# richarddurbin/modimizer

Hardware: AMD Instinct MI355X
Metric: Gbp/s hashed+sketched (k=21,d=64) (higher is better)
Workload: dtype u64; 1 GPU; BASELINE config 2: 10 Gbp synthetic ONT-like reads (log-normal N50 20 kb, 5% subs, 30x of a 333 Mbp genome), k=21 d=64 seed=17, seqhash scan + modset build (table bits 30); reads_per_gpu=598835, bases_per_gpu=10000000000, modimizers_per_gpu=156043826, modset_entries=102967436, k=21, d=64, table_bits=30, parallelism=reads sharded x1, modset per GPU

## Files before the change

### modimizer_amd/csrc/mg_api.hip

```cpp
#include <stdarg.h>
#include <stdlib.h>
#include <string.h>
#include <mutex>
#include <unordered_map>
#include "mg_common.h"
#include "mg_internal.h"
#include "mg_xfer.h"


static thread_local char gErr[512] = "";

void mgSetError (const char *fmt, ...)
{ va_list ap; va_start (ap, fmt); vsnprintf (gErr, sizeof (gErr), fmt, ap); va_end (ap); }

extern "C" const char *mgLastError (void) { return gErr; }

MgStatus mgHipFail (hipError_t e, const char *what)
{ mgSetError ("HIP error %d (%s) in %s", (int) e, hipGetErrorString (e), what); return MG_ERR_HIP; }

extern "C" int mgDeviceCount (void)
{ int n = 0; if (hipGetDeviceCount (&n) != hipSuccess) { (void) hipGetLastError (); return 0; } return n; }

MgStatus mgEnsureDevice (void)
{
// ... 430 lines not shown
static std::unordered_map<const Modset *, MgDev *> gReg;
extern "C" { volatile int mgLiveDeviceModsets = 0; }

static MgDev *mgDevLookup (const Modset *ms)
{ std::lock_guard<std::mutex> g (gRegLock); auto it = gReg.find (ms); return it == gReg.end () ? 0 : it->second; }

static void mgDevFree (MgDev *d)
{
  if (!d) return;
  MgOnDevice here (d->device);
  if (d->hPin) (void) hipHostFree (d->hPin);
  if (d->built)
    { (void) hipFree (d->t.slots); (void) hipFree (d->t.value); (void) hipFree (d->t.occ); (void) hipFree (d->t.find8);
      (void) hipFree (d->t.baseDepth); (void) hipFree (d->t.counters); (void) hipFree (d->t.liveHist);
    }
  if (d->side) { (void) hipStreamSynchronize (d->side); (void) hipStreamDestroy (d->side); }
  d->arena.release (); d->arena2.release ();
  for (int i = 0 ; i < 2 ; ++i) if (d->scanned[i]) (void) hipEventDestroy (d->scanned[i]);
  if (d->inputReady) (void) hipEventDestroy (d->inputReady);
  delete d;
}

#define MG_LOOKUP_LOAD_PCT 40
static MgStatus mgDevBuild (Modset *ms, MgDev *d, hipStream_t st)
{
  MgTable &t = d->t;
  if (ms->tableBits < 20 || ms->tableBits > 32)
    { mgSetError ("device modset supports table bits 20..32 (got %d)", ms->tableBits); return MG_ERR_ARG; }
  memset (&t, 0, sizeof (t));
  t.maxLog2Slots = ms->tableBits - 1;
  t.kbits = 2 * ms->hasher->k;
  t.wantR = 4096;
  { const long r = mgKnobs ()->bucketR; if (r != MG_KNOB_UNSET && r >= 256) t.wantR = (U32) r; }
  t.size = ms->size;
  t.pin = d->hPin + 24;
  U64 cap = (ms->tableSize >> 2);
  MG_HIP (hipMalloc ((void **) &t.value, cap * sizeof (U64)));
  MG_HIP (hipMalloc ((void **) &t.baseDepth, cap * sizeof (U16)));
  MG_HIP (hipMalloc ((void **) &t.counters, 64));
  d->built = true;
  MG_HIP (hipMemsetAsync (t.baseDepth, 0, cap * sizeof (U16), st));
  MG_HIP (hipMemsetAsync (t.counters, 0, 64, st));
  { MgStatus s0 = mgTableEnsure (&t, ms->max, st); if (s0) return s0; }
  t.max = 0; t.syncedMax = 0;
  t.baseZero = !ms->max;
  if (ms->max)
    { MG_HIP (hipStreamSynchronize (st));
      MgStatus s;
      if ((s = mgXferH2D (t.value, ms->value, ((size_t) ms->max + 1) * sizeof (U64)))) return s;
      if ((s = mgXferH2D (t.baseDepth, ms->depth, ((size_t) ms->max + 1) * sizeof (U16)))) return s;
      if ((s = mgTableLoadHost (&t, t.value, 1, ms->max, st))) return s;
      MG_HIP (hipStreamSynchronize (st));
      t.max = t.syncedMax = ms->max;
    }
  d->hostIndexMax = ms->max;
// ... 208 lines not shown

static U64 mgAddChunkSize (void)
{
  const long c = mgKnobs ()->addChunk;
  U64 v = c != MG_KNOB_UNSET && c > 0 ? (U64) c : ((U64) 1 << 30);
  if (v > ((U64) 1 << 30)) v = (U64) 1 << 30;
  return v;
}
#define MG_ADD_CHUNK (mgAddChunkSize ())

static MgStatus mgAddChunk (Modset *ms, MgDev *d, const U64 *dKmer, U64 n, U32 *dIndexOut, int withDepth,
                            void *scratch, hipStream_t st, const MgHistReq *counted = 0, const MgSegSrc *segSrc = 0)
{
  MgTable &t = d->t;
  MgStatus s;
  MG_HIP (hipMemsetAsync (t.counters, 0, 16, st));
  if ((s = mgTableAdd (&t, dKmer, n, withDepth, scratch, st, counted, segSrc))) return s;
  volatile U64 *c = d->hPin;
  MG_HIP (hipMemcpyAsync (d->hPin, t.counters, 16, hipMemcpyDeviceToHost, st));
  MG_HIP (hipStreamSynchronize (st));
  U64 newMax = (U64) t.max + c[0];
  if (c[1] || newMax >= t.size)
    {
      if ((s = mgTableRollback (&t, st))) return s;
      mgSetError ("hashTableSize %u is too small for %llu", t.size, (unsigned long long) newMax);
      return MG_ERR_CAPACITY;
    }
  t.max = (U32) newMax;
  ms->max = t.max;
  if (n >= 4096) t.newPct = (int) (c[0] * 100 / n);
  if (dIndexOut && (s = mgTableFind (&t, dKmer, n, dIndexOut, st))) return s;
// ... 634 lines not shown
```

### modimizer_amd/csrc/mg_common.h

```cpp
#ifndef MG_COMMON_H
#define MG_COMMON_H
#include "mg_knobs.h"

#include <hip/hip_runtime.h>
#include <stdint.h>
#include <time.h>
#include <algorithm>
#include <vector>
#include "modgpu.h"

#define MG_WAVE 64

#define MG_SCAN_THREADS   256
#define MG_POS_PER_THREAD 64
#define MG_TILE_BASES     (64 * MG_POS_PER_THREAD)
#define MG_TILE_WORDS     (MG_TILE_BASES / 16)

struct MgHashParams {
  U64 factor1;
  U64 mask;
  int k;
  int shift1;
  U32 d;
  int dShift;
// ... 184 lines not shown
  U32 syncedMax;
  U64 *counters;
  bool pendingDepth;
  bool dirty;
  U64 *find8;
  U64 find8Cap;
  U64 find8Version, version;
  bool empty;
  U64 *pin;
  int newPct;
  int loadPct;
  int  maxLog2Slots;
  U32  wantR;
  U64  diag[7];
  int  tightPct;
};
MgStatus mgTableAlloc (MgTable *t, U64 slotsWanted, hipStream_t st);
MgStatus mgTableEnsure (MgTable *t, U64 nIncoming, hipStream_t st);
MgStatus mgTableRollback (MgTable *t, hipStream_t st);
MgStatus mgTableClean (MgTable *t, hipStream_t st);
void     mgTableForget (MgTable *t, hipStream_t st);
size_t   mgTableAddScratchBytes (const MgTable *t, U64 n);
bool     mgTableUseBuckets (const MgTable *t, U64 n);
MgStatus mgTableAdd (MgTable *t, const U64 *dKmer, U64 n, int withDepth, void *scratch, hipStream_t st,
                     const MgHistReq *counted = 0,
                     const MgSegSrc *segSrc = 0);
bool     mgTableAddTakesSegments (const MgTable *t, U64 n, const MgHistReq *counted);
MgStatus mgTableMarkOccupied (MgTable *t, const U64 *dKmer, U64 n, hipStream_t st);
MgStatus mgTableFind (MgTable *t, const U64 *dKmer, U64 n, U32 *dIndexOut, hipStream_t st);
MgStatus mgTableLayoutCheck (MgTable *t, U64 *dOut4, hipStream_t st);
enum { MG_DIAG_FIND_DIRECT = 0, MG_DIAG_FIND_PART1, MG_DIAG_FIND_PART2_16, MG_DIAG_FIND_PART2_8, MG_DIAG_PACK8, MG_DIAG_REHASH_BUCKET, MG_DIAG_REHASH_ATOMIC };
// ... 24 lines not shown
```

### modimizer_amd/csrc/mg_knobs.c

```c
#define _GNU_SOURCE
#include <pthread.h>
#include <sched.h>
#include <stdio.h>
#include <stdlib.h>
#include <string.h>
#include <unistd.h>
#include <sys/mman.h>
#include "mg_knobs.h"

static MgKnobs gKnobs;
static pthread_once_t gOnce = PTHREAD_ONCE_INIT;

static long num (const char *name)
{ const char *e = getenv (name); return e && *e ? atol (e) : MG_KNOB_UNSET; }

static void readAll (void)
{
  MgKnobs k;
  const char *e = getenv ("MODGPU_TABLE_PATH");
  k.tablePath = e && *e ? (long) e[0] : MG_KNOB_UNSET;
  e = getenv ("MODGPU_FIND_PATH");
  k.findPath = e && *e ? (long) e[0] : MG_KNOB_UNSET;
  k.partPacked = num ("MODGPU_PART_PACKED");       k.partBig = num ("MODGPU_PART_BIG");
  k.addChunk = num ("MODGPU_ADD_CHUNK");           k.scanGrid = num ("MODGPU_SCAN_GRID");
  k.scanGeneric = num ("MODGPU_SCAN_GENERIC");     k.scanHist = num ("MODGPU_SCAN_HIST");
  k.scanDiv64 = num ("MODGPU_SCAN_DIV64");        k.minTiled = num ("MODGPU_MIN_TILED");
  k.minTile = num ("MODGPU_MIN_TILE");
  k.noSegmentInput = num ("MODGPU_NO_SEGMENT_INPUT");
  k.rankSliceShift = num ("MODGPU_RANK_SLICE_SHIFT");
  k.flagPolarity = num ("MODGPU_FLAG_POLARITY");   k.mergeSlots = num ("MODGPU_MERGE_SLOTS");
  k.mergePlace = num ("MODGPU_MERGE_PLACE");
  k.bucketR = num ("MODGPU_BUCKET_R");             k.bucketT = num ("MODGPU_BUCKET_T");
  e = getenv ("MODGPU_HOT_SPLIT");
  k.hotSplit = e && *e ? atol (e) : MG_KNOB_UNSET;
  { const char *c = e ? strchr (e, ',') : 0; k.hotChunk = c ? atol (c + 1) : MG_KNOB_UNSET; }
  k.noAvx2 = num ("MODGPU_NO_AVX2");               k.textHost = num ("MODGPU_TEXT_HOST");
  k.textWindowKb = num ("MODGPU_TEXT_WINDOW_KB");
  k.fileBatchMbp = num ("MODGPU_FILE_BATCH_MBP");  k.fileBatchBases = num ("MODGPU_FILE_BATCH_BASES");
  k.queryHostChain = num ("MODGPU_QUERY_HOST_CHAIN");
  k.iterHostBelow = num ("MODGPU_ITER_HOST_BELOW");
  k.readsetHost = num ("MODGPU_READSET_HOST");
  k.segSlack = num ("MODGPU_SEG_SLACK");
  k.partDigits = num ("MODGPU_PART_DIGITS");
  k.findBits = num ("MODGPU_FIND_BITS");
  k.scatterGrid = num ("MODGPU_SCATTER_GRID");     k.tableLoad = num ("MODGPU_TABLE_LOAD");
  k.tightLoad = num ("MODGPU_TIGHT_LOAD");         k.find8 = num ("MODGPU_FIND8");
// ... 44 lines not shown
```

### modimizer_amd/csrc/mg_knobs.h

```cpp
#ifndef MG_KNOBS_H
#define MG_KNOBS_H
#include <limits.h>
#ifdef __cplusplus
extern "C" {
#endif
#define MG_KNOB_UNSET LONG_MIN
typedef struct {
  long findPath;
  long tablePath;
  long partPacked;
  long partBig;
  long addChunk;
  long scanGrid;
  long scanGeneric;
  long minTile;
  long minTiled;
  long scanDiv64;
  long scanHist;
  long noSegmentInput;
  long rankSliceShift;
  long flagPolarity;
  long mergeSlots;
  long mergePlace;
  long bucketR, bucketT;
  long hotSplit, hotChunk;
  long noAvx2;
  long textHost;
  long textWindowKb;
  long fileBatchMbp;
  long fileBatchBases;
  long readsetHost;
  long queryHostChain;
  long iterHostBelow;
  long scatterGrid;
  long segSlack;
  long partDigits;
  long findBits;
  long tableLoad;
// ... 22 lines not shown
```

### modimizer_amd/csrc/mg_scan.hip

```cpp
#include <stdlib.h>
#include "mg_prefix.h"


__global__ void mgPackKernel (const U8 *__restrict__ bases, U64 nBases, U32 *__restrict__ words, U64 nWords)
{
  U64 i = (U64) blockIdx.x * blockDim.x + threadIdx.x;
  U64 stride = (U64) gridDim.x * blockDim.x;
  const bool aligned = (((uintptr_t) bases) & 15) == 0;
  for ( ; i < nWords ; i += stride)
    { U64 b0 = i * 16;
      U32 w = 0;
      if (b0 + 16 <= nBases && aligned)
        { uint4 v = *reinterpret_cast<const uint4 *> (bases + b0);
          U32 q[4] = { v.x, v.y, v.z, v.w };
#pragma unroll
          for (int j = 0 ; j < 4 ; ++j)
            { U32 x = q[j];
              U32 n = ((x & 3) << 6) | (((x >> 8) & 3) << 4) | (((x >> 16) & 3) << 2) | ((x >> 24) & 3);
              w |= n << (24 - 8 * j);
            }
        }
      else if (b0 < nBases)
        { for (int j = 0 ; j < 16 && b0 + j < nBases ; ++j)
            w |= (U32) (bases[b0 + j] & 3) << (30 - 2 * j);
// ... 466 lines not shown
  for (int w = 0 ; w < MG_ITER_WAVES ; ++w) { const U64 v = sFound[w]; if (w < wave) before += v; total += v; }
  if (total <= o.capEntries)
    { U32 *posOut = reinterpret_cast<U32 *> (o.out + 1 + total);
      const U64 src = (U64) wave * a.segCap;
      for (U64 i = (U64) lane ; i < found ; i += 64)
        { o.out[1 + before + i] = a.segKmer[src + i];
          posOut[before + i] = a.segPosF[src + i];
        }
    }
  if (threadIdx.x == 0) o.out[0] = total;
  __threadfence_system ();
  __syncthreads ();
  if (threadIdx.x == 0) __hip_atomic_store (const_cast<U64 *> (o.flag), o.seq, __ATOMIC_RELEASE, __HIP_MEMORY_SCOPE_SYSTEM);
}

__global__ __launch_bounds__ (1024)
void mgSegScanKernel (const U64 *__restrict__ blockCount, U32 nBlocks, U64 segCap, U64 capacity,
                      U64 *__restrict__ segStart, U64 *__restrict__ dCount)
{
  __shared__ U64 sV[8192 + 1024];
  __shared__ U64 sWaveSum[16], sWaveMax[16];
  const int tid = threadIdx.x, lane = tid & 63, wave = tid >> 6;
  U64 carry = 0, gmx = 0;
  for (U32 base = 0 ; base < nBlocks ; base += 8192)
    {
#pragma unroll
      for (int j = 0 ; j < 8 ; ++j)
        { U32 e = (U32) j * 1024 + tid, b = base + e;
          sV[e + (e >> 3)] = b < nBlocks ? blockCount[b] : 0;
        }
      __syncthreads ();
      U64 c[8], sum = 0, mx = 0;
#pragma unroll
      for (int j = 0 ; j < 8 ; ++j) { c[j] = sV[tid * 9 + j]; sum += c[j]; if (c[j] > mx) mx = c[j]; }
      U64 incl = sum, wmx = mx;
#pragma unroll
      for (int off = 1 ; off < 64 ; off <<= 1)
        { U32 lo = __shfl_up ((U32) incl, off), hi = __shfl_up ((U32) (incl >> 32), off);
          if (lane >= off) incl += ((U64) hi << 32) | lo;
          U32 ml = __shfl_xor ((U32) wmx, off), mh = __shfl_xor ((U32) (wmx >> 32), off);
          U64 o = ((U64) mh << 32) | ml; if (o > wmx) wmx = o;
        }
      if (lane == 63) { sWaveSum[wave] = incl; sWaveMax[wave] = wmx; }
      __syncthreads ();
      U64 before = 0, total = 0;
#pragma unroll
      for (int w = 0 ; w < 16 ; ++w) { U64 v = sWaveSum[w]; if (w < wave) before += v; total += v; if (sWaveMax[w] > gmx) gmx = sWaveMax[w]; }
      U64 run = carry + before + incl - sum;
#pragma unroll
      for (int j = 0 ; j < 8 ; ++j) { sV[tid * 9 + j] = run; run += c[j]; }
      __syncthreads ();
#pragma unroll
      for (int j = 0 ; j < 8 ; ++j)
        { U32 e = (U32) j * 1024 + tid, b = base + e;
          if (b < nBlocks) segStart[b] = sV[e + (e >> 3)];
        }
      carry += total;
      __syncthreads ();
    }
  if (tid == 0)
    { segStart[nBlocks] = carry;
      dCount[0] = carry;
      dCount[1] = (gmx > segCap || carry > capacity) ? 1 : 0;
      dCount[2] = gmx;
      U64 need = gmx * (U64) nBlocks;
      dCount[3] = need > carry ? need : carry;
    }
}

__global__ __launch_bounds__ (256)
void mgSegCompactKernel (const U64 *__restrict__ segKmer, const U32 *__restrict__ segPosF,
                         const U32 *__restrict__ segRead, U64 segCap, U32 nSegs,
                         const U64 *__restrict__ blockCount, const U64 *__restrict__ segStart,
// ... 152 lines not shown
  const bool scanCounts = histEnv && hist && hist->binCount && hist->kbits >= 24 && hHiB >= 1 && hHiB <= MG_MIX_TOP && hLoB + hHiB == hist->log2NB;
  a.histCount = scanCounts ? hist->binCount : 0; a.histKbits = hist ? hist->kbits : 64; a.histHiB = hHiB;
#ifdef MG_ABLATE
  { const long dbg = mgKnobs ()->scanDebug; a.debug = dbg != MG_KNOB_UNSET ? (U32) dbg : 0u; }
#endif
  const unsigned grid = (g.nBlocks + MG_WAVES - 1) / MG_WAVES;
  const int mode = mgScanMode (p, &a);
  const bool where = a.segPosF || a.segRead;
#define MG_SCAN_LAUNCH(M) do { if (where) MG_LAUNCH (MG_K_SCAN, st, (mgScanKernel<M, true>), dim3 (grid), dim3 (MG_SCAN_THREADS), 0, st, a); \
                               else       MG_LAUNCH (MG_K_SCAN, st, (mgScanKernel<M, false>), dim3 (grid), dim3 (MG_SCAN_THREADS), 0, st, a); } while (0)
  if (mode == MG_MODE_FAST) MG_SCAN_LAUNCH (MG_MODE_FAST); else if (mode == MG_MODE_POW2) MG_SCAN_LAUNCH (MG_MODE_POW2);
  else if (mode == MG_MODE_ODD) MG_SCAN_LAUNCH (MG_MODE_ODD); else if (mode == MG_MODE_ODD32) MG_SCAN_LAUNCH (MG_MODE_ODD32);
  else if (mode == MG_MODE_ANY32) MG_SCAN_LAUNCH (MG_MODE_ANY32); else MG_SCAN_LAUNCH (MG_MODE_ANY);
#undef MG_SCAN_LAUNCH
  MG_HIP (hipGetLastError ());
  MG_LAUNCH (MG_K_SEG_SCAN, st, mgSegScanKernel, dim3 (1), dim3 (1024), 0, st, blockCount, g.nBlocks, g.segCap, capacity, segStart, dCount);
  MG_HIP (hipGetLastError ());
  { int hiB = 0, loB = 0; U32 bins = 0;
    if (hist && hist->binCount && !scanCounts) { mgPartSplit (hist->log2NB, &hiB, &loB); bins = (U32) 1 << hiB; }
    const unsigned cgrid = g.nBlocks < 4096 ? g.nBlocks : 4096;
    if (lazy) { lazy->segKmer = segKmer; lazy->segCount = blockCount; lazy->segStart = segStart; lazy->segCap = g.segCap; lazy->nSegs = g.nBlocks; }
    if (!lazy || bins || dPosF || dReadId)
      MG_LAUNCH (MG_K_SEG_COMPACT, st, mgSegCompactKernel, dim3 (cgrid), dim3 (256), 0, st,
                 segKmer, a.segPosF, a.segRead, g.segCap, g.nBlocks, blockCount, segStart, lazy ? (U64 *) 0 : dKmer, dPosF, dReadId, capacity, dCount,
                 hist ? hist->log2NB : 0, hist ? hist->kbits : 64, loB, bins, hist ? hist->binCount : (U32 *) 0);
  }
  MG_HIP (hipGetLastError ());
  return MG_OK;
}

MgStatus mgLaunchSegCompact (const MgSegSrc &src, U64 *dKmer, U64 capacity, const U64 *dCount, hipStream_t st)
// ... 55 lines not shown
```

### modimizer_amd/csrc/mg_table.hip

```cpp
#include <stdlib.h>
#include <string.h>
#include "mg_prefix.h"

#define MG_ASSIGNED 0x80000000u
#define MG_R_QUANTUM 64u
#ifdef MG_BUILD_PRIO
#define MG_BUILD_PRIO() __builtin_amdgcn_s_setprio (3)
#else
#define MG_BUILD_PRIO() do { } while (0)
#endif
#ifdef MG_ABLATE
#define MG_ABLATE_AND(x) && (x)
#else
#define MG_ABLATE_AND(x)
#endif
__device__ __forceinline__ U32 mgToken (U64 o) { return 0x7fffffffu - (U32) o; }
__device__ __forceinline__ bool mgIsAssigned (U32 v) { return (v & MG_ASSIGNED) != 0; }
__device__ __forceinline__ U64 mgKeyOf (const uint4 &v) { return ((U64) v.y << 32) | v.x; }
__device__ __forceinline__ U32 mgIndexOf (U32 ordWord) { return mgIsAssigned (ordWord) ? (ordWord & ~MG_ASSIGNED) : 0; }
__device__ __forceinline__ bool mgLiveEntry (const uint4 &v, U32 keepMax) { return (v.x | v.y) && mgIsAssigned (v.z) && (v.z & ~MG_ASSIGNED) <= keepMax; }




// ... 702 lines not shown
          if (dOut) dOut[at] = (unsigned char) mgDigitOf<(PACKOUT ? MG_EL_PACKED : MG_EL_WIDE)> (stK[p], g, f, dShift, dMask);
        }
      __syncthreads ();
      c = nc; seg = nseg; lo = nlo; hi = nhi; sub = nsub; have = nhave;
    }
}



struct MgBucketArgs {
  MgSlot *slots; MgGeom g; U32 nBuckets;
  const U64 *bucketStart;
  U64 *pK; U32 *pT; U32 *pC;
  MgPartFmt f;
  U32 *uniqCount;
  U32 *occ;
  unsigned char *flags;
  const MgRankGrp *grp; U32 baseMax; U32 size;
  unsigned short *sliceOff;
  U32 nSlices; int sliceShift;
  int slotShift;
  int place;
  int markDup;
  int withDepth;
  U64 *counters;
  U32 hotSplit, hotChunk;
  U64 *hotItems; unsigned long long *hotCount;
  U32 *hotBuckets;
#ifdef MG_ABLATE
  int debug;
// ... 240 lines not shown
    }
}

template <bool PACKED, bool SLOT, int PER, bool HOT>
__global__ __launch_bounds__ (1024) __attribute__ ((amdgpu_waves_per_eu (PER == MG_DEDUP_PER ? 8 : 4)))
void mgBucketDedupKernel (const MgBucketArgs a, U32 bucketsPerBlock)
{
  MG_BUILD_PRIO ();
  const U32 R = a.g.R, T = blockDim.x, tid = threadIdx.x;
  unsigned long long *sKey = reinterpret_cast<unsigned long long *> (mgDynLds);
  U32 *sOrd = reinterpret_cast<U32 *> (mgDynLds + (size_t) R * 8);
  U32 *sCnt = sOrd + R;
  U32 *sGrp = sCnt + R;
  const U32 nGrp = a.nSlices + 1;
  U32 b = blockIdx.x * bucketsPerBlock, bEnd = b + bucketsPerBlock;
  U64 hotAt = blockIdx.x; const U64 nHot = HOT ? a.hotCount[1] : 0;
  if (HOT) { if (hotAt >= nHot) return; }
  else
    { if (bEnd > a.nBuckets) bEnd = a.nBuckets;
      if (b >= bEnd) return;
    }
  for (U32 i = tid ; i < R ; i += T) { sKey[i] = 0; sOrd[i] = 0; sCnt[i] = 0; }
  if (tid < MG_RANK_GROUPS) sGrp[tid] = 0;
  for ( ; ; )
  {
  if (HOT) { b = a.hotBuckets[hotAt]; bEnd = b + 1; }
  U64 lo = a.bucketStart[b], hi = a.bucketStart[b + 1];
  U32 occNow = a.occ[b];
  U64 ck[MG_BUCKET_PREFETCH]; U32 ct[MG_BUCKET_PREFETCH];
#pragma unroll
// ... 55 lines not shown
              rk[j] = 0; rc[j] = 0; ro[j] = 0; rp[j] = 0;
              if (i < R) rk[j] = sKey[i];
              if (rk[j])
                { rc[j] = sCnt[i]; ro[j] = sOrd[i];
                  sKey[i] = 0; sOrd[i] = 0; sCnt[i] = 0;
                  rk[j] = (rk[j] - 1) | (SLOT ? (unsigned long long) i << MG_SLOT_SHIFT : 0ull);
                  if (rc[j]) rp[j] = atomicAdd (&sGrp[mgIsAssigned (ro[j]) ? a.nSlices : ((0x7fffffffu - ro[j]) >> a.sliceShift)], 1u);
                }
            }
          __syncthreads ();
          const int lane = (int) (tid & 63);
          const U32 gv = (U32) lane < nGrp ? sGrp[lane] : 0;
          const U32 gIncl = mgWaveInclusiveSum (gv);
          const U32 gBase = gIncl - gv;
          const U32 total = (U32) __builtin_amdgcn_readlane ((int) gIncl, 63);
          if (tid < 64)
            { if ((U32) lane <= nGrp) a.sliceOff[(U64) b * (nGrp + 1) + lane] = (unsigned short) gBase;
              if (lane == 0) a.uniqCount[b] = total;
            }
#pragma unroll
          for (int j = 0 ; j < PER ; ++j)
            { const U32 grp = mgIsAssigned (ro[j]) ? a.nSlices : ((0x7fffffffu - ro[j]) >> a.sliceShift);
              const U32 at = (U32) __shfl ((int) gBase, (int) (rc[j] ? grp : 0)) + rp[j];
              if (rc[j]) { sKey[at] = rk[j]; sOrd[at] = ro[j]; sCnt[at] = rc[j]; }
            }
          __syncthreads ();
          if (tid < MG_RANK_GROUPS) sGrp[tid] = 0;
          for (U32 i = tid ; i < total ; i += T)
            { const U64 k = sKey[i]; const U32 ord = sOrd[i], c = sCnt[i];
              sKey[i] = 0; sOrd[i] = 0; sCnt[i] = 0;
              if (true MG_ABLATE_AND (!(a.debug & 8)))
                { __builtin_nontemporal_store (k, &a.pK[lo + i]); __builtin_nontemporal_store (ord, &a.pT[lo + i]); __builtin_nontemporal_store (c, &a.pC[lo + i]); }
              if (!a.markDup && !mgIsAssigned (ord) MG_ABLATE_AND (!(a.debug & 1))) a.flags[0x7fffffffu - ord] = 1;
            }
          __syncthreads ();
        }
      lo = nlo; hi = nhi; occNow = occNext;
#pragma unroll
      for (int j = 0 ; j < MG_BUCKET_PREFETCH ; ++j) { ck[j] = nk[j]; ct[j] = nt[j]; }
    }
  if (!HOT) break;
  hotAt += gridDim.x;
  if (hotAt >= nHot) break;
  }
}

__device__ __forceinline__ U32 mgPlaceStarts (U32 *cnt, unsigned short *sStart, int *sWave, U32 R, U32 T, U32 tid, U32 n)
{
  const U32 per = (R + 4 * T - 1) / (4 * T) * 4;
  const U32 j0 = tid * per, j1 = j0 + per < R ? j0 + per : R;
  U32 vS = 0; int vM = 0;
  for (U32 j = j0 ; j < j1 ; j += 4)
    { const uint4 c = *reinterpret_cast<const uint4 *> (&cnt[j]);
      int m = (int) j - (int) vS;               vM = m > vM ? m : vM; vS += c.x;
      m = (int) (j + 1) - (int) vS;             vM = m > vM ? m : vM; vS += c.y;
      m = (int) (j + 2) - (int) vS;             vM = m > vM ? m : vM; vS += c.z;
      m = (int) (j + 3) - (int) vS;             vM = m > vM ? m : vM; vS += c.w;
    }
  const int lane = (int) (tid & 63);
// ... 826 lines not shown
#undef MG_SCATTER_P
#undef MG_SCATTER
  MG_HIP (hipGetLastError ());
  return MG_OK;
}

__global__ __launch_bounds__ (256)
void mgUniqStatsKernel (const U32 *__restrict__ uniqCount, U32 nBuckets, unsigned long long *__restrict__ out)
{
  unsigned long long sum = 0; U32 mx = 0;
  for (U32 b = blockIdx.x * 256 + threadIdx.x ; b < nBuckets ; b += gridDim.x * 256) { const U32 c = uniqCount[b]; sum += c; mx = c > mx ? c : mx; }
  sum = mgWaveReduce<MgSum> ((U64) sum); mx = mgWaveReduce<MgMax> (mx);
  if ((threadIdx.x & 63) == 0) { if (sum) atomicAdd (&out[0], sum); if (mx) atomicMax (&out[1], (unsigned long long) mx); }
}

#define MG_TIGHT_PCT_DEFAULT 70
#define MG_TIGHT_PCT_CLAIMS 50
#define MG_TIGHT_MIN_R 1024u

MgStatus mgTableAdd (MgTable *t, const U64 *dKmer, U64 n, int withDepth, void *scratch, hipStream_t st,
                     const MgHistReq *counted, const MgSegSrc *segSrc)
{
  if (!n) return MG_OK;
  if (segSrc && !mgTableAddTakesSegments (t, n, counted)) { mgSetError ("internal: this insert needs the dense k-mers"); return MG_ERR_ARG; }
  const MgSegSrc noSrc = {};
  t->liveHistValid = false;
  if (withDepth) t->pendingDepth = true;
  const bool wasEmpty = t->empty && t->max == 0;
  t->empty = false; ++t->version;
  MgGeom g = mgGeomOf (t);
  char *wb = (char *) scratch;
  unsigned char *flags = (unsigned char *) wb;       wb += mgAl256 (n);
  U64 *blockCount = (U64 *) wb;                      wb += mgAl256 ((MG_RANK_UNITS + 8) * 8);
  U64 *blockBase = (U64 *) wb;                       wb += mgAl256 ((MG_RANK_UNITS + 8) * 8);
  MgRankGrp *grp = (MgRankGrp *) wb;                 wb += mgAl256 ((n / 64 + 2) * sizeof (MgRankGrp));
  U32 nRankBlocks; U64 rankTiles = mgRankRowsPerUnit (n, &nRankBlocks);
  MG_HIP (hipMemsetAsync (blockCount, 0, (MG_RANK_UNITS + 8) * 8, st));

  if (!mgTableUseBuckets (t, n))
    { U32 *slotId = (U32 *) wb;
      { MgStatus cs = mgTableClean (t, st); if (cs) return cs; }
      MG_LAUNCH (MG_K_TABLE_INSERT, st, mgTableInsertKernel, dim3 (mgGridWide (n)), dim3 (256), 0, st, t->slots, g, dKmer, n, slotId, withDepth, t->counters);
      MG_LAUNCH (MG_K_TABLE_FLAG, st, mgDirectFlagKernel, dim3 (mgGridWide (n)), dim3 (256), 0, st, t->slots, slotId, n, flags);
      MG_LAUNCH (MG_K_RANK_COUNT, st, mgRankCountKernel, dim3 (nRankBlocks), dim3 (256), 0, st, flags, n, rankTiles, blockCount);
      MG_LAUNCH (MG_K_RANK_SCAN, st, (mgGroupSumKernel<U64, U64>), dim3 (1), dim3 (MG_GROUP_THREADS), 0, st, blockCount, blockBase, nRankBlocks * 4, t->counters);
      MG_LAUNCH (MG_K_TABLE_ASSIGN, st, (mgRankAssignKernel<true, false>), dim3 (nRankBlocks), dim3 (256), 0, st,
                 flags, dKmer, noSrc, (const MgSubSeg *) 0, n, rankTiles, blockBase, t->max, t->size, t->value, t->slots, slotId, grp);
      MG_HIP (hipGetLastError ());
      return mgTableMarkOccupied (t, dKmer, n, st);
    }

  const U64 NB = (U64) 1 << t->log2NB;
// ... 11 lines not shown
  unsigned long long *coarseCursor = (unsigned long long *) wb; wb += mgAl256 (((U64) MG_PART_MAXBINS + 2) * 8 * 16);
  U64 *whole = (U64 *) wb;                    wb += mgAl256 (((U64) MG_PART_MAXBINS + 2) * 8);
  U32 *coarseCount = (U32 *) wb;              wb += mgAl256 ((MG_PART_MAXBINS + 2) * 4);
  U32 *chunkBase = (U32 *) wb;                wb += mgAl256 ((MG_PART_MAXBINS + 2 + n / MG_PART_CHUNK + MG_PART_MAXBINS + 2) * 4);
  unsigned short *sliceOff = (unsigned short *) wb;   wb += mgAl256 ((size_t) (MG_RANK_GROUPS + 2) * NB * sizeof (unsigned short));
  MgSubSeg *subSeg = (MgSubSeg *) wb;         wb += mgAl256 ((n / MG_PART_SUB + 2) * sizeof (MgSubSeg));
  U64 *hotItems = (U64 *) wb;                 wb += mgAl256 (mgHotItemsCap (n) * 8);
  U32 *hotBuckets = (U32 *) wb;               wb += mgAl256 (mgHotItemsCap (n) * 4);
  unsigned long long *hotCount = (unsigned long long *) wb; wb += 256;
  (void) spare64;

  const int j = t->log2NB;
  int hiB, loB;
  mgPartSplit (j, &hiB, &loB);
  const U32 *pre = (counted && counted->binCount && counted->log2NB == j && counted->kbits == t->kbits && !counted->hiB) ? counted->binCount : 0;
  U64 segInit[2] = { 0, n };
  MG_HIP (hipMemcpyAsync (whole, segInit, 16, hipMemcpyHostToDevice, st));
  const MgPartFmt f = mgPartFmtOf (t, n, hiB);
  const int packEnv = mgKnobs ()->partPacked == MG_KNOB_UNSET ? 1 : (int) mgKnobs ()->partPacked;
  const bool packed = packEnv && mgPartFmtFits (t, f);
  MgStatus s;
  const U64 *bucketStart = fineStart;
  MgPartPassArgs p1 = {};
  p1.inMode = segSrc ? MG_EL_SEG : MG_EL_DENSE; p1.packed = packed; p1.f = f; p1.kIn = dKmer; p1.n = n; p1.segStart = whole; p1.nSeg = 1;
  p1.nBins = (U32) 1 << hiB; p1.chunkBase = chunkBase; p1.counted = pre; p1.segSrc = segSrc; p1.subSeg = subSeg;
  if (!loB)
    { p1.kOut = kB; p1.tOut = tB; p1.binStart = fineStart; p1.cursor = fineCursor; p1.binCount = fineCount;
      if ((s = mgPartPass (t, p1, st))) return s;
    }
  else
    {
      unsigned char *digits = (loB <= 8 && mgKnobs ()->partDigits != 0) ? reinterpret_cast<unsigned char *> (cB) : 0;
      p1.shift = loB; p1.kOut = kA; p1.tOut = tA; p1.binStart = coarseStart; p1.cursor = coarseCursor; p1.binCount = coarseCount;
      p1.digitOut = digits; p1.nextBins = (U32) 1 << loB;
      if ((s = mgPartPass (t, p1, st))) return s;
      MgPartPassArgs p2 = {};
      p2.inMode = packed ? MG_EL_PACKED : MG_EL_WIDE; p2.packed = packed; p2.f = f; p2.kIn = kA; p2.tIn = tA; p2.n = n; p2.segStart = coarseStart; p2.nSeg = (U32) 1 << hiB;
      p2.nBins = (U32) 1 << loB; p2.kOut = kB; p2.tOut = tB; p2.binStart = fineStart; p2.cursor = fineCursor; p2.binCount = fineCount; p2.chunkBase = chunkBase;
      p2.digitIn = digits;
      if ((s = mgPartPass (t, p2, st))) return s;
    }

  MgBucketArgs a;
  { const int polEnv = mgKnobs ()->flagPolarity == MG_KNOB_UNSET ? -1 : (int) mgKnobs ()->flagPolarity;
    a.markDup = polEnv >= 0 ? (polEnv ? 1 : 0) : (t->newPct > 50 ? 1 : 0);
  }
  MG_HIP (hipMemsetAsync (flags, a.markDup ? 1 : 0, n, st));
  const U64 expectNew = t->newPct > 0 ? n * (U64) t->newPct / 100 : n;
  { const int slotEnv = mgKnobs ()->mergeSlots == MG_KNOB_UNSET ? -1 : (int) mgKnobs ()->mergeSlots;
    const bool dense = ((U64) t->max + expectNew) * 2 > t->nSlots;
    a.slotShift = (t->kbits <= MG_SLOT_SHIFT && (slotEnv >= 0 ? slotEnv != 0 : dense)) ? MG_SLOT_SHIFT : 0;
  }
  int tightPct = t->tightPct ? t->tightPct : MG_TIGHT_PCT_CLAIMS;
  { const long tk = mgKnobs ()->tightLoad; if (tk != MG_KNOB_UNSET && tk >= 0 && tk <= 95) tightPct = (int) tk; }
  bool tighten = wasEmpty && tightPct > 0 && t->log2NB > 0 && t->pin;
  if (tighten && mgKnobs ()->tightLoad == MG_KNOB_UNSET)
    tighten = expectNew * 100 / (U64) tightPct < t->nSlots - t->nSlots / 4;
  { const long pk = mgKnobs ()->mergePlace;
// ... 8 lines not shown
  if (tighten) a.slotShift = 0;
  a.slots = t->slots; a.g = g; a.nBuckets = (U32) NB; a.bucketStart = bucketStart;
  a.pK = kB; a.pT = tB; a.pC = cB; a.uniqCount = uniqCount; a.occ = t->occ; a.flags = flags;
  a.grp = grp; a.baseMax = t->max; a.size = t->size; a.withDepth = withDepth;
  { a.sliceShift = 22;
    while (a.sliceShift > 16 && ((n - 1) >> a.sliceShift) + 1 < 32) --a.sliceShift;
    if (mgKnobs ()->rankSliceShift != MG_KNOB_UNSET) a.sliceShift = (int) mgKnobs ()->rankSliceShift;
    while (((n - 1) >> a.sliceShift) + 1 > (U64) (MG_RANK_GROUPS - 1)) ++a.sliceShift;
    a.nSlices = (U32) (((n - 1) >> a.sliceShift) + 1);
    a.sliceOff = sliceOff;
  }
  a.counters = t->counters; a.f = f;
#ifdef MG_ABLATE
  { const long dbg = mgKnobs ()->bucketDebug; a.debug = dbg != MG_KNOB_UNSET ? (int) dbg : 0; }
#endif
  const bool track = t->max == 0 && t->baseZero;
  a.liveHist = 0;
  if (track)
    { if (!t->liveHist) MG_HIP (hipMalloc ((void **) &t->liveHist, 65536 * sizeof (U64)));
      MG_HIP (hipMemsetAsync (t->liveHist, 0, 65536 * sizeof (U64), st));
      a.liveHist = (unsigned long long *) t->liveHist;
    }
  t->liveHistValid = track;
  size_t lds = mgMergeLdsBytes (t->R);
  { const size_t ldsDedup = (size_t) t->R * 16 + MG_RANK_GROUPS * 4; if (ldsDedup > lds) lds = ldsDedup; }
  const bool bigR = t->R > MG_DEDUP_PER * 1024u;
  if (t->R > MG_DEDUP_PER_BIG * 1024u) { mgSetError ("internal: bucket of %u slots", t->R); return MG_ERR_ARG; }
  if (lds > 48 * 1024)
    {
#define MG_DEDUP_ATTR(PK, SL, PER) do { MG_HIP (hipFuncSetAttribute ((const void *) mgBucketDedupKernel<PK, SL, PER, false>, hipFuncAttributeMaxDynamicSharedMemorySize, (int) lds)); \
                                        MG_HIP (hipFuncSetAttribute ((const void *) mgBucketDedupKernel<PK, SL, PER, true>, hipFuncAttributeMaxDynamicSharedMemorySize, (int) lds)); } while (0)
      if (bigR) { MG_DEDUP_ATTR (true, true, MG_DEDUP_PER_BIG); MG_DEDUP_ATTR (true, false, MG_DEDUP_PER_BIG); MG_DEDUP_ATTR (false, true, MG_DEDUP_PER_BIG); MG_DEDUP_ATTR (false, false, MG_DEDUP_PER_BIG); }
      else      { MG_DEDUP_ATTR (true, true, MG_DEDUP_PER); MG_DEDUP_ATTR (true, false, MG_DEDUP_PER); MG_DEDUP_ATTR (false, true, MG_DEDUP_PER); MG_DEDUP_ATTR (false, false, MG_DEDUP_PER); }
#undef MG_DEDUP_ATTR
      MG_HIP (hipFuncSetAttribute ((const void *) mgBucketMergeKernel<MG_MERGE_PREFETCH>, hipFuncAttributeMaxDynamicSharedMemorySize, (int) lds));
      MG_HIP (hipFuncSetAttribute ((const void *) mgBucketMergeKernel<MG_PLACE_KEEP>, hipFuncAttributeMaxDynamicSharedMemorySize, (int) lds));
    }
  const int bThreadsEnv = mgKnobs ()->bucketT == MG_KNOB_UNSET ? 0 : (int) mgKnobs ()->bucketT;
  const unsigned bThreads = mgBucketThreads (t->R, bThreadsEnv);
  U32 perBlock;
  const unsigned bGrid = mgBucketGrid (NB, &perBlock);
  if ((U64) bThreads * (bigR ? MG_DEDUP_PER_BIG : MG_DEDUP_PER) < t->R)
    { mgSetError ("internal: %u threads for a bucket of %u slots", bThreads, t->R); return MG_ERR_ARG; }
  mgHotKnobs (&a.hotSplit, &a.hotChunk);
  a.hotItems = hotItems; a.hotCount = hotCount; a.hotBuckets = hotBuckets;
  MG_HIP (hipMemsetAsync (hotCount, 0, 16, st));
  MG_LAUNCH (MG_K_HOT_REDUCE, st, mgHotPlanKernel, dim3 ((unsigned) ((NB + 255) / 256)), dim3 (256), 0, st, a);
  { const size_t ldsHot = (size_t) t->R * 16 + 16;
    if (packed) { if (ldsHot > 48 * 1024) MG_HIP (hipFuncSetAttribute ((const void *) mgHotReduceKernel<true>, hipFuncAttributeMaxDynamicSharedMemorySize, (int) ldsHot));
                  MG_LAUNCH (MG_K_HOT_REDUCE, st, mgHotReduceKernel<true>, dim3 (1024), dim3 (bThreads), ldsHot, st, a); }
    else        { if (ldsHot > 48 * 1024) MG_HIP (hipFuncSetAttribute ((const void *) mgHotReduceKernel<false>, hipFuncAttributeMaxDynamicSharedMemorySize, (int) ldsHot));
                  MG_LAUNCH (MG_K_HOT_REDUCE, st, mgHotReduceKernel<false>, dim3 (1024), dim3 (bThreads), ldsHot, st, a); }
  }
#define MG_DEDUP_LAUNCH(PK, SL, PER) do { MG_LAUNCH (MG_K_BUCKET_DEDUP, st, (mgBucketDedupKernel<PK, SL, PER, false>), dim3 (bGrid), dim3 (bThreads), lds, st, a, perBlock); \
                                          MG_LAUNCH (MG_K_HOT_REDUCE, st, (mgBucketDedupKernel<PK, SL, PER, true>), dim3 (64), dim3 (bThreads), lds, st, a, perBlock); } while (0)
#define MG_DEDUP_PICK(PER) do { if (packed) { if (a.slotShift) MG_DEDUP_LAUNCH (true, true, PER); else MG_DEDUP_LAUNCH (true, false, PER); } \
                                else        { if (a.slotShift) MG_DEDUP_LAUNCH (false, true, PER); else MG_DEDUP_LAUNCH (false, false, PER); } } while (0)
  if (bigR) MG_DEDUP_PICK (MG_DEDUP_PER_BIG); else MG_DEDUP_PICK (MG_DEDUP_PER);
#undef MG_DEDUP_PICK
#undef MG_DEDUP_LAUNCH
  U64 fullest = t->R;
  if (tighten)
    { unsigned long long *st2 = (unsigned long long *) (t->counters + 2);
      MG_HIP (hipMemsetAsync (st2, 0, 16, st));
      MG_LAUNCH (MG_K_RANK_SCAN, st, mgUniqStatsKernel, dim3 ((unsigned) (NB / 256 < 256 ? (NB + 255) / 256 : 256)), dim3 (256), 0, st, uniqCount, (U32) NB, st2);
      MG_HIP (hipMemcpyAsync (t->pin, t->counters + 1, 24, hipMemcpyDeviceToHost, st));
      MG_HIP (hipStreamSynchronize (st));
      const U64 over = t->pin[0], U = t->pin[1], M = t->pin[2];
      if (!over)
        { fullest = M;
          U64 Rn = (U * 100 / ((U64) NB * (U64) tightPct) + 1 + MG_R_QUANTUM - 1) / MG_R_QUANTUM * MG_R_QUANTUM;
          const U64 Rfit = (M + M / 8 + 16 + MG_R_QUANTUM - 1) / MG_R_QUANTUM * MG_R_QUANTUM;
          if (Rn < Rfit) Rn = Rfit;
          if (Rn < MG_TIGHT_MIN_R) Rn = MG_TIGHT_MIN_R;
          if (Rn < t->R)
            { t->R = (U32) Rn; t->nSlots = (U64) NB * Rn; a.g = mgGeomOf (t);
              lds = mgMergeLdsBytes (t->R);
            }
        }
    }
  MG_LAUNCH (MG_K_RANK_COUNT, st, mgRankCountKernel, dim3 (nRankBlocks), dim3 (256), 0, st, flags, n, rankTiles, blockCount);
  MG_LAUNCH (MG_K_RANK_SCAN, st, (mgGroupSumKernel<U64, U64>), dim3 (1), dim3 (MG_GROUP_THREADS), 0, st, blockCount, blockBase, nRankBlocks * 4, t->counters);
  if (segSrc)
    MG_LAUNCH (MG_K_TABLE_ASSIGN, st, (mgRankAssignKernel<false, true>), dim3 (nRankBlocks), dim3 (256), 0, st,
               flags, (const U64 *) 0, *segSrc, subSeg, n, rankTiles, blockBase, t->max, t->size, t->value, t->slots, (const U32 *) 0, grp);
  else
    MG_LAUNCH (MG_K_TABLE_ASSIGN, st, (mgRankAssignKernel<false, false>), dim3 (nRankBlocks), dim3 (256), 0, st,
               flags, dKmer, noSrc, (const MgSubSeg *) 0, n, rankTiles, blockBase, t->max, t->size, t->value, t->slots, (const U32 *) 0, grp);
  { const U32 groupsPerSlice = (U32) ((NB + 63) / 64);
    const U32 blocksPerSlice = (groupsPerSlice + 3) / 4, rounds = (a.nSlices + 7) / 8;
    MG_LAUNCH (MG_K_RANK_LOOKUP, st, mgRankLookupKernel, dim3 (8 * rounds * blocksPerSlice), dim3 (256), 0, st, a, groupsPerSlice);
  }
  if (fullest <= (U64) MG_MERGE_PREFETCH * bThreads)
    MG_LAUNCH (MG_K_BUCKET_MERGE, st, mgBucketMergeKernel<MG_MERGE_PREFETCH>, dim3 (bGrid), dim3 (bThreads), lds, st, a, perBlock);
  else
    MG_LAUNCH (MG_K_BUCKET_MERGE, st, mgBucketMergeKernel<MG_PLACE_KEEP>, dim3 (bGrid), dim3 (bThreads), lds, st, a, perBlock);
  MG_HIP (hipGetLastError ());
  return MG_OK;
}

__global__ void mgMarkOccKernel (MgGeom g, const U64 *__restrict__ kmer, U64 n, U32 *__restrict__ occ)
{
  U64 o = (U64) blockIdx.x * blockDim.x + threadIdx.x;
// ... 357 lines not shown
```

Measured before the change: 1239 Gbp/s.

## Chain modset build launches: fuse init memsets, overlap host sync with rank pass

Adds a buildChain knob that, when set, replaces several small memsets and an H2D copy with one init kernel. It folds unique-count stats into the dedup kernel instead of a separate stats kernel. It also launches the rank pass before waiting on an event for the pinned stats, so the host sync overlaps GPU work. The segment scan kernel gains a prefetching, grouped variant. The knob defaults to unset, which is nonzero, so the chained path runs by default. The cost is more code paths, and the rank pass now runs before R is tightened; this is valid only if it does not depend on R.

```diff
diff --git a/modimizer_amd/csrc/mg_api.hip b/modimizer_amd/csrc/mg_api.hip
--- a/modimizer_amd/csrc/mg_api.hip
+++ b/modimizer_amd/csrc/mg_api.hip
@@ -468,6 +468,7 @@
     { (void) hipFree (d->t.slots); (void) hipFree (d->t.value); (void) hipFree (d->t.occ); (void) hipFree (d->t.find8);
       (void) hipFree (d->t.baseDepth); (void) hipFree (d->t.counters); (void) hipFree (d->t.liveHist);
     }
+  mgTableSyncDrop (&d->t);
   if (d->side) { (void) hipStreamSynchronize (d->side); (void) hipStreamDestroy (d->side); }
   d->arena.release (); d->arena2.release ();
   for (int i = 0 ; i < 2 ; ++i) if (d->scanned[i]) (void) hipEventDestroy (d->scanned[i]);
@@ -493,6 +494,7 @@
   MG_HIP (hipMalloc ((void **) &t.baseDepth, cap * sizeof (U16)));
   MG_HIP (hipMalloc ((void **) &t.counters, 64));
   d->built = true;
+  { MgStatus s0 = mgTableSyncMake (&t); if (s0) return s0; }
   MG_HIP (hipMemsetAsync (t.baseDepth, 0, cap * sizeof (U16), st));
   MG_HIP (hipMemsetAsync (t.counters, 0, 64, st));
   { MgStatus s0 = mgTableEnsure (&t, ms->max, st); if (s0) return s0; }
@@ -731,7 +733,6 @@
 {
   MgTable &t = d->t;
   MgStatus s;
-  MG_HIP (hipMemsetAsync (t.counters, 0, 16, st));
   if ((s = mgTableAdd (&t, dKmer, n, withDepth, scratch, st, counted, segSrc))) return s;
   volatile U64 *c = d->hPin;
   MG_HIP (hipMemcpyAsync (d->hPin, t.counters, 16, hipMemcpyDeviceToHost, st));
diff --git a/modimizer_amd/csrc/mg_common.h b/modimizer_amd/csrc/mg_common.h
--- a/modimizer_amd/csrc/mg_common.h
+++ b/modimizer_amd/csrc/mg_common.h
@@ -222,7 +222,10 @@
   U32  wantR;
   U64  diag[7];
   int  tightPct;
-};
+  hipEvent_t pinFilled;
+};
+MgStatus mgTableSyncMake (MgTable *t);
+void     mgTableSyncDrop (MgTable *t);
 MgStatus mgTableAlloc (MgTable *t, U64 slotsWanted, hipStream_t st);
 MgStatus mgTableEnsure (MgTable *t, U64 nIncoming, hipStream_t st);
 MgStatus mgTableRollback (MgTable *t, hipStream_t st);
diff --git a/modimizer_amd/csrc/mg_knobs.c b/modimizer_amd/csrc/mg_knobs.c
--- a/modimizer_amd/csrc/mg_knobs.c
+++ b/modimizer_amd/csrc/mg_knobs.c
@@ -29,7 +29,7 @@
   k.noSegmentInput = num ("MODGPU_NO_SEGMENT_INPUT");
   k.rankSliceShift = num ("MODGPU_RANK_SLICE_SHIFT");
   k.flagPolarity = num ("MODGPU_FLAG_POLARITY");   k.mergeSlots = num ("MODGPU_MERGE_SLOTS");
-  k.mergePlace = num ("MODGPU_MERGE_PLACE");
+  k.mergePlace = num ("MODGPU_MERGE_PLACE");       k.buildChain = num ("MODGPU_BUILD_CHAIN");
   k.bucketR = num ("MODGPU_BUCKET_R");             k.bucketT = num ("MODGPU_BUCKET_T");
   e = getenv ("MODGPU_HOT_SPLIT");
   k.hotSplit = e && *e ? atol (e) : MG_KNOB_UNSET;
diff --git a/modimizer_amd/csrc/mg_knobs.h b/modimizer_amd/csrc/mg_knobs.h
--- a/modimizer_amd/csrc/mg_knobs.h
+++ b/modimizer_amd/csrc/mg_knobs.h
@@ -22,6 +22,7 @@
   long flagPolarity;
   long mergeSlots;
   long mergePlace;
+  long buildChain;
   long bucketR, bucketT;
   long hotSplit, hotChunk;
   long noAvx2;
diff --git a/modimizer_amd/csrc/mg_scan.hip b/modimizer_amd/csrc/mg_scan.hip
--- a/modimizer_amd/csrc/mg_scan.hip
+++ b/modimizer_amd/csrc/mg_scan.hip
@@ -504,6 +504,8 @@
   if (threadIdx.x == 0) __hip_atomic_store (const_cast<U64 *> (o.flag), o.seq, __ATOMIC_RELEASE, __HIP_MEMORY_SCOPE_SYSTEM);
 }
 
+#define MG_SEG_GROUP 2
+template <int G, bool AHEAD>
 __global__ __launch_bounds__ (1024)
 void mgSegScanKernel (const U64 *__restrict__ blockCount, U32 nBlocks, U64 segCap, U64 capacity,
                       U64 *__restrict__ segStart, U64 *__restrict__ dCount)
@@ -512,41 +514,66 @@
   __shared__ U64 sWaveSum[16], sWaveMax[16];
   const int tid = threadIdx.x, lane = tid & 63, wave = tid >> 6;
   U64 carry = 0, gmx = 0;
-  for (U32 base = 0 ; base < nBlocks ; base += 8192)
+  U64 v[G][8], nx[G][8];
+  auto fetch = [&] (U64 (&to)[G][8], U32 from)
     {
 #pragma unroll
-      for (int j = 0 ; j < 8 ; ++j)
-        { U32 e = (U32) j * 1024 + tid, b = base + e;
-          sV[e + (e >> 3)] = b < nBlocks ? blockCount[b] : 0;
-        }
-      __syncthreads ();
-      U64 c[8], sum = 0, mx = 0;
-#pragma unroll
-      for (int j = 0 ; j < 8 ; ++j) { c[j] = sV[tid * 9 + j]; sum += c[j]; if (c[j] > mx) mx = c[j]; }
-      U64 incl = sum, wmx = mx;
-#pragma unroll
-      for (int off = 1 ; off < 64 ; off <<= 1)
-        { U32 lo = __shfl_up ((U32) incl, off), hi = __shfl_up ((U32) (incl >> 32), off);
-          if (lane >= off) incl += ((U64) hi << 32) | lo;
-          U32 ml = __shfl_xor ((U32) wmx, off), mh = __shfl_xor ((U32) (wmx >> 32), off);
-          U64 o = ((U64) mh << 32) | ml; if (o > wmx) wmx = o;
-        }
-      if (lane == 63) { sWaveSum[wave] = incl; sWaveMax[wave] = wmx; }
-      __syncthreads ();
-      U64 before = 0, total = 0;
-#pragma unroll
-      for (int w = 0 ; w < 16 ; ++w) { U64 v = sWaveSum[w]; if (w < wave) before += v; total += v; if (sWaveMax[w] > gmx) gmx = sWaveMax[w]; }
-      U64 run = carry + before + incl - sum;
-#pragma unroll
-      for (int j = 0 ; j < 8 ; ++j) { sV[tid * 9 + j] = run; run += c[j]; }
-      __syncthreads ();
-#pragma unroll
-      for (int j = 0 ; j < 8 ; ++j)
-        { U32 e = (U32) j * 1024 + tid, b = base + e;
-          if (b < nBlocks) segStart[b] = sV[e + (e >> 3)];
-        }
-      carry += total;
-      __syncthreads ();
+      for (int r = 0 ; r < G ; ++r)
+#pragma unroll
+        for (int j = 0 ; j < 8 ; ++j)
+          { const U32 b = from + (U32) r * 8192 + (U32) j * 1024 + tid;
+            to[r][j] = b < nBlocks ? blockCount[b] : 0;
+          }
+    };
+  if (AHEAD) fetch (v, 0);
+  for (U32 first = 0 ; first < nBlocks ; first += (U32) G * 8192)
+    {
+      if (AHEAD) fetch (nx, first + (U32) G * 8192); else fetch (v, first);
+#pragma unroll
+      for (int r = 0 ; r < G ; ++r)
+        { const U32 base = first + (U32) r * 8192;
+          if (base >= nBlocks) break;
+#pragma unroll
+          for (int j = 0 ; j < 8 ; ++j)
+            { U32 e = (U32) j * 1024 + tid;
+              sV[e + (e >> 3)] = v[r][j];
+            }
+          __syncthreads ();
+          U64 c[8], sum = 0, mx = 0;
+#pragma unroll
+          for (int j = 0 ; j < 8 ; ++j) { c[j] = sV[tid * 9 + j]; sum += c[j]; if (c[j] > mx) mx = c[j]; }
+          U64 incl = sum, wmx = mx;
+#pragma unroll
+          for (int off = 1 ; off < 64 ; off <<= 1)
+            { U32 lo = __shfl_up ((U32) incl, off), hi = __shfl_up ((U32) (incl >> 32), off);
+              if (lane >= off) incl += ((U64) hi << 32) | lo;
+              U32 ml = __shfl_xor ((U32) wmx, off), mh = __shfl_xor ((U32) (wmx >> 32), off);
+              U64 o = ((U64) mh << 32) | ml; if (o > wmx) wmx = o;
+            }
+          if (lane == 63) { sWaveSum[wave] = incl; sWaveMax[wave] = wmx; }
+          __syncthreads ();
+          U64 before = 0, total = 0;
+#pragma unroll 2
+          for (int w = 0 ; w < 16 ; ++w) { U64 x = sWaveSum[w]; if (w < wave) before += x; total += x; if (sWaveMax[w] > gmx) gmx = sWaveMax[w]; }
+          U64 run = carry + before + incl - sum;
+#pragma unroll
+          for (int j = 0 ; j < 8 ; ++j) { sV[tid * 9 + j] = run; run += c[j]; }
+          __syncthreads ();
+#pragma unroll
+          for (int j = 0 ; j < 8 ; ++j)
+            { U32 e = (U32) j * 1024 + tid, b = base + e;
+              if (b < nBlocks) segStart[b] = sV[e + (e >> 3)];
+            }
+          carry += total;
+          __syncthreads ();
+        }
+      if (AHEAD)
+        {
+#pragma unroll
+          for (int r = 0 ; r < G ; ++r)
+#pragma unroll
+            for (int j = 0 ; j < 8 ; ++j) v[r][j] = nx[r][j];
+        }
     }
   if (tid == 0)
     { segStart[nBlocks] = carry;
@@ -729,7 +756,10 @@
   else if (mode == MG_MODE_ANY32) MG_SCAN_LAUNCH (MG_MODE_ANY32); else MG_SCAN_LAUNCH (MG_MODE_ANY);
 #undef MG_SCAN_LAUNCH
   MG_HIP (hipGetLastError ());
-  MG_LAUNCH (MG_K_SEG_SCAN, st, mgSegScanKernel, dim3 (1), dim3 (1024), 0, st, blockCount, g.nBlocks, g.segCap, capacity, segStart, dCount);
+  if (mgKnobs ()->buildChain != 0)
+    MG_LAUNCH (MG_K_SEG_SCAN, st, (mgSegScanKernel<MG_SEG_GROUP, true>), dim3 (1), dim3 (1024), 0, st, blockCount, g.nBlocks, g.segCap, capacity, segStart, dCount);
+  else
+    MG_LAUNCH (MG_K_SEG_SCAN, st, (mgSegScanKernel<1, false>), dim3 (1), dim3 (1024), 0, st, blockCount, g.nBlocks, g.segCap, capacity, segStart, dCount);
   MG_HIP (hipGetLastError ());
   { int hiB = 0, loB = 0; U32 bins = 0;
     if (hist && hist->binCount && !scanCounts) { mgPartSplit (hist->log2NB, &hiB, &loB); bins = (U32) 1 << hiB; }
diff --git a/modimizer_amd/csrc/mg_table.hip b/modimizer_amd/csrc/mg_table.hip
--- a/modimizer_amd/csrc/mg_table.hip
+++ b/modimizer_amd/csrc/mg_table.hip
@@ -740,6 +740,7 @@
   U64 *pK; U32 *pT; U32 *pC;
   MgPartFmt f;
   U32 *uniqCount;
+  unsigned long long *uniqStats;
   U32 *occ;
   unsigned char *flags;
   const MgRankGrp *grp; U32 baseMax; U32 size;
@@ -1010,6 +1011,7 @@
   U32 *sGrp = sCnt + R;
   const U32 nGrp = a.nSlices + 1;
   U32 b = blockIdx.x * bucketsPerBlock, bEnd = b + bucketsPerBlock;
+  U32 uSum = 0, uMax = 0;
   U64 hotAt = blockIdx.x; const U64 nHot = HOT ? a.hotCount[1] : 0;
   if (HOT) { if (hotAt >= nHot) return; }
   else
@@ -1095,6 +1097,7 @@
           const U32 gIncl = mgWaveInclusiveSum (gv);
           const U32 gBase = gIncl - gv;
           const U32 total = (U32) __builtin_amdgcn_readlane ((int) gIncl, 63);
+          uSum += total; uMax = total > uMax ? total : uMax;
           if (tid < 64)
             { if ((U32) lane <= nGrp) a.sliceOff[(U64) b * (nGrp + 1) + lane] = (unsigned short) gBase;
               if (lane == 0) a.uniqCount[b] = total;
@@ -1124,6 +1127,7 @@
   hotAt += gridDim.x;
   if (hotAt >= nHot) break;
   }
+  if (a.uniqStats && tid == 0 && uSum) { atomicAdd (&a.uniqStats[0], (unsigned long long) uSum); atomicMax (&a.uniqStats[1], (unsigned long long) uMax); }
 }
 
 __device__ __forceinline__ U32 mgPlaceStarts (U32 *cnt, unsigned short *sStart, int *sWave, U32 R, U32 T, U32 tid, U32 n)
@@ -1980,6 +1984,23 @@
   if ((threadIdx.x & 63) == 0) { if (sum) atomicAdd (&out[0], sum); if (mx) atomicMax (&out[1], (unsigned long long) mx); }
 }
 
+__global__ __launch_bounds__ (256)
+void mgAddInitKernel (U64 *__restrict__ counters, U64 *__restrict__ blockCount, U32 nBlockCount, unsigned long long *__restrict__ hotCount,
+                      U64 *__restrict__ whole, U64 n, unsigned long long *__restrict__ liveHist)
+{
+  const U32 i = blockIdx.x * 256 + threadIdx.x, stride = gridDim.x * 256;
+  if (i < 4) counters[i] = 0;
+  if (i < 2) { hotCount[i] = 0; whole[i] = i ? n : 0; }
+  for (U32 j = i ; j < nBlockCount ; j += stride) blockCount[j] = 0;
+  if (liveHist) for (U32 j = i ; j < 65536 ; j += stride) liveHist[j] = 0;
+}
+
+MgStatus mgTableSyncMake (MgTable *t)
+{ MG_HIP (hipEventCreateWithFlags (&t->pinFilled, hipEventDisableTiming)); return MG_OK; }
+
+void mgTableSyncDrop (MgTable *t)
+{ if (t->pinFilled) { (void) hipEventDestroy (t->pinFilled); t->pinFilled = 0; } }
+
 #define MG_TIGHT_PCT_DEFAULT 70
 #define MG_TIGHT_PCT_CLAIMS 50
 #define MG_TIGHT_MIN_R 1024u
@@ -2001,7 +2022,11 @@
   U64 *blockBase = (U64 *) wb;                       wb += mgAl256 ((MG_RANK_UNITS + 8) * 8);
   MgRankGrp *grp = (MgRankGrp *) wb;                 wb += mgAl256 ((n / 64 + 2) * sizeof (MgRankGrp));
   U32 nRankBlocks; U64 rankTiles = mgRankRowsPerUnit (n, &nRankBlocks);
-  MG_HIP (hipMemsetAsync (blockCount, 0, (MG_RANK_UNITS + 8) * 8, st));
+  const bool chain = mgKnobs ()->buildChain != 0 && mgTableUseBuckets (t, n);
+  if (!chain)
+    { MG_HIP (hipMemsetAsync (t->counters, 0, 16, st));
+      MG_HIP (hipMemsetAsync (blockCount, 0, (MG_RANK_UNITS + 8) * 8, st));
+    }
 
   if (!mgTableUseBuckets (t, n))
     { U32 *slotId = (U32 *) wb;
@@ -2043,8 +2068,19 @@
   int hiB, loB;
   mgPartSplit (j, &hiB, &loB);
   const U32 *pre = (counted && counted->binCount && counted->log2NB == j && counted->kbits == t->kbits && !counted->hiB) ? counted->binCount : 0;
-  U64 segInit[2] = { 0, n };
-  MG_HIP (hipMemcpyAsync (whole, segInit, 16, hipMemcpyHostToDevice, st));
+  MgBucketArgs a;
+  const bool track = t->max == 0 && t->baseZero;
+  a.liveHist = 0;
+  if (track)
+    { if (!t->liveHist) MG_HIP (hipMalloc ((void **) &t->liveHist, 65536 * sizeof (U64)));
+      a.liveHist = (unsigned long long *) t->liveHist;
+    }
+  if (chain)
+    MG_LAUNCH (MG_K_MEMSET, st, mgAddInitKernel, dim3 (64), dim3 (256), 0, st, t->counters, blockCount, (U32) (MG_RANK_UNITS + 8), hotCount, whole, n, a.liveHist);
+  else
+    { U64 segInit[2] = { 0, n };
+      MG_HIP (hipMemcpyAsync (whole, segInit, 16, hipMemcpyHostToDevice, st));
+    }
   const MgPartFmt f = mgPartFmtOf (t, n, hiB);
   const int packEnv = mgKnobs ()->partPacked == MG_KNOB_UNSET ? 1 : (int) mgKnobs ()->partPacked;
   const bool packed = packEnv && mgPartFmtFits (t, f);
@@ -2070,7 +2106,6 @@
       if ((s = mgPartPass (t, p2, st))) return s;
     }
 
-  MgBucketArgs a;
   { const int polEnv = mgKnobs ()->flagPolarity == MG_KNOB_UNSET ? -1 : (int) mgKnobs ()->flagPolarity;
     a.markDup = polEnv >= 0 ? (polEnv ? 1 : 0) : (t->newPct > 50 ? 1 : 0);
   }
@@ -2109,13 +2144,7 @@
 #ifdef MG_ABLATE
   { const long dbg = mgKnobs ()->bucketDebug; a.debug = dbg != MG_KNOB_UNSET ? (int) dbg : 0; }
 #endif
-  const bool track = t->max == 0 && t->baseZero;
-  a.liveHist = 0;
-  if (track)
-    { if (!t->liveHist) MG_HIP (hipMalloc ((void **) &t->liveHist, 65536 * sizeof (U64)));
-      MG_HIP (hipMemsetAsync (t->liveHist, 0, 65536 * sizeof (U64), st));
-      a.liveHist = (unsigned long long *) t->liveHist;
-    }
+  if (track && !chain) MG_HIP (hipMemsetAsync (t->liveHist, 0, 65536 * sizeof (U64), st));
   t->liveHistValid = track;
   size_t lds = mgMergeLdsBytes (t->R);
   { const size_t ldsDedup = (size_t) t->R * 16 + MG_RANK_GROUPS * 4; if (ldsDedup > lds) lds = ldsDedup; }
@@ -2139,7 +2168,8 @@
     { mgSetError ("internal: %u threads for a bucket of %u slots", bThreads, t->R); return MG_ERR_ARG; }
   mgHotKnobs (&a.hotSplit, &a.hotChunk);
   a.hotItems = hotItems; a.hotCount = hotCount; a.hotBuckets = hotBuckets;
-  MG_HIP (hipMemsetAsync (hotCount, 0, 16, st));
+  a.uniqStats = tighten && chain ? (unsigned long long *) (t->counters + 2) : 0;
+  if (!chain) MG_HIP (hipMemsetAsync (hotCount, 0, 16, st));
   MG_LAUNCH (MG_K_HOT_REDUCE, st, mgHotPlanKernel, dim3 ((unsigned) ((NB + 255) / 256)), dim3 (256), 0, st, a);
   { const size_t ldsHot = (size_t) t->R * 16 + 16;
     if (packed) { if (ldsHot > 48 * 1024) MG_HIP (hipFuncSetAttribute ((const void *) mgHotReduceKernel<true>, hipFuncAttributeMaxDynamicSharedMemorySize, (int) ldsHot));
@@ -2157,10 +2187,26 @@
   U64 fullest = t->R;
   if (tighten)
     { unsigned long long *st2 = (unsigned long long *) (t->counters + 2);
-      MG_HIP (hipMemsetAsync (st2, 0, 16, st));
-      MG_LAUNCH (MG_K_RANK_SCAN, st, mgUniqStatsKernel, dim3 ((unsigned) (NB / 256 < 256 ? (NB + 255) / 256 : 256)), dim3 (256), 0, st, uniqCount, (U32) NB, st2);
+      if (!chain)
+        { MG_HIP (hipMemsetAsync (st2, 0, 16, st));
+          MG_LAUNCH (MG_K_RANK_SCAN, st, mgUniqStatsKernel, dim3 ((unsigned) (NB / 256 < 256 ? (NB + 255) / 256 : 256)), dim3 (256), 0, st, uniqCount, (U32) NB, st2);
+        }
       MG_HIP (hipMemcpyAsync (t->pin, t->counters + 1, 24, hipMemcpyDeviceToHost, st));
-      MG_HIP (hipStreamSynchronize (st));
+      if (chain) MG_HIP (hipEventRecord (t->pinFilled, st));
+    }
+  auto rankPass = [&] ()
+    { MG_LAUNCH (MG_K_RANK_COUNT, st, mgRankCountKernel, dim3 (nRankBlocks), dim3 (256), 0, st, flags, n, rankTiles, blockCount);
+      MG_LAUNCH (MG_K_RANK_SCAN, st, (mgGroupSumKernel<U64, U64>), dim3 (1), dim3 (MG_GROUP_THREADS), 0, st, blockCount, blockBase, nRankBlocks * 4, t->counters);
+      if (segSrc)
+        MG_LAUNCH (MG_K_TABLE_ASSIGN, st, (mgRankAssignKernel<false, true>), dim3 (nRankBlocks), dim3 (256), 0, st,
+                   flags, (const U64 *) 0, *segSrc, subSeg, n, rankTiles, blockBase, t->max, t->size, t->value, t->slots, (const U32 *) 0, grp);
+      else
+        MG_LAUNCH (MG_K_TABLE_ASSIGN, st, (mgRankAssignKernel<false, false>), dim3 (nRankBlocks), dim3 (256), 0, st,
+                   flags, dKmer, noSrc, (const MgSubSeg *) 0, n, rankTiles, blockBase, t->max, t->size, t->value, t->slots, (const U32 *) 0, grp);
+    };
+  if (chain) rankPass ();
+  if (tighten)
+    { if (chain) MG_HIP (hipEventSynchronize (t->pinFilled)); else MG_HIP (hipStreamSynchronize (st));
       const U64 over = t->pin[0], U = t->pin[1], M = t->pin[2];
       if (!over)
         { fullest = M;
@@ -2174,14 +2220,7 @@
             }
         }
     }
-  MG_LAUNCH (MG_K_RANK_COUNT, st, mgRankCountKernel, dim3 (nRankBlocks), dim3 (256), 0, st, flags, n, rankTiles, blockCount);
-  MG_LAUNCH (MG_K_RANK_SCAN, st, (mgGroupSumKernel<U64, U64>), dim3 (1), dim3 (MG_GROUP_THREADS), 0, st, blockCount, blockBase, nRankBlocks * 4, t->counters);
-  if (segSrc)
-    MG_LAUNCH (MG_K_TABLE_ASSIGN, st, (mgRankAssignKernel<false, true>), dim3 (nRankBlocks), dim3 (256), 0, st,
-               flags, (const U64 *) 0, *segSrc, subSeg, n, rankTiles, blockBase, t->max, t->size, t->value, t->slots, (const U32 *) 0, grp);
-  else
-    MG_LAUNCH (MG_K_TABLE_ASSIGN, st, (mgRankAssignKernel<false, false>), dim3 (nRankBlocks), dim3 (256), 0, st,
-               flags, dKmer, noSrc, (const MgSubSeg *) 0, n, rankTiles, blockBase, t->max, t->size, t->value, t->slots, (const U32 *) 0, grp);
+  if (!chain) rankPass ();
   { const U32 groupsPerSlice = (U32) ((NB + 63) / 64);
     const U32 blocksPerSlice = (groupsPerSlice + 3) / 4, rounds = (a.nSlices + 7) / 8;
     MG_LAUNCH (MG_K_RANK_LOOKUP, st, mgRankLookupKernel, dim3 (8 * rounds * blocksPerSlice), dim3 (256), 0, st, a, groupsPerSlice);
```

Result: no change. 1246 Gbp/s (median of 6 runs) (+0.6%).
